# daxiongpro/EPNet

Measured on AMD Instinct MI355X. Metric: SA-stack points/sec per GPU (16384-pt KITTI scene) + % HBM roofline, higher is better.
Workload: dtype f32

## Files before the change

### epnet_amd/_lib.py

```python
import contextlib
import ctypes
import os

_HERE = os.path.dirname(os.path.abspath(__file__))
LIB_PATH = os.environ.get("EPNET_HIP_LIB") or os.path.join(_HERE, "lib", "libepnet_hip.so")

_vp = ctypes.c_void_p
_i = ctypes.c_int
_f = ctypes.c_float
_d = ctypes.c_double
_sz = ctypes.c_size_t
_i64 = ctypes.c_int64

SIGNATURES = {
    "epnet_abi_version": (_i, []),
    "epnet_strerror": (ctypes.c_char_p, [_i]),
    "epnet_last_hip_error": (ctypes.c_char_p, []),
    "epnet_set_tuning": (_i, [ctypes.c_char_p, _i]),
    "epnet_get_tuning": (_i, [ctypes.c_char_p, ctypes.POINTER(_i)]),
    "epnet_furthest_point_sampling": (_i, [_i, _i, _i, _vp, _vp, _vp, _vp]),
    "epnet_gather_points": (_i, [_i, _i, _i, _i, _vp, _vp, _vp, _vp]),
    "epnet_gather_points_grad": (_i, [_i, _i, _i, _i, _vp, _vp, _vp, _vp]),
    "epnet_ball_query": (_i, [_i, _i, _i, _f, _i, _vp, _vp, _vp, _vp]),
    "epnet_ball_query_workspace_bytes": (_sz, [_i, _i, _i]),
# ... 28 lines not shown
    "epnet_three_interpolate_grad_det": (_i, [_i, _i, _i, _i, _vp, _vp, _vp, _vp, _vp, _sz, _vp]),
    "epnet_feature_gather_grad_det_workspace_bytes": (_sz, [_i, _i, _i, _i]),
    "epnet_feature_gather_grad_det": (_i, [_i, _i, _i, _i, _i, _i, _vp, _vp, _vp, _vp, _sz, _vp]),
    "epnet_group_linear_grad_w_det_workspace_bytes": (_sz, [_i, _i, _i, _i]),
    "epnet_group_linear_grad_w_det": (_i, [_i, _i, _i, _i, _i, _vp, _vp, _vp, _vp, _vp, _vp, _sz, _vp]),
    "epnet_pool_max": (_i, [ctypes.c_longlong, _i, _vp, _vp, _vp, _vp]),
    "epnet_pool_max_grad": (_i, [ctypes.c_longlong, _i, _vp, _vp, _vp, _vp]),
    "epnet_scene_index_bytes": (_sz, [_i, _i]),
    "epnet_scene_index_build": (_i, [_i, _i, _vp, _vp, _sz, _vp]),
    "epnet_scene_index_build_gathered": (_i, [_i, _i, _i, _vp, _vp, _vp, _vp, _sz, _vp]),
    "epnet_furthest_point_sampling_indexed": (_i, [_i, _i, _i, _vp, _vp, _sz, _vp, _vp, _vp]),
    "epnet_sample_centres": (_i, [_i, _i, _i, _vp, _vp, _sz, _vp, _vp, _vp, _vp]),
    "epnet_sample_centres_chain": (_i, [_i, _i, _i, _vp, _vp, _sz, _vp, _vp, _vp, _vp, _vp, _i, _vp]),
    "epnet_group_concat_multi": (_i, [_i, _i, _i, _i, _i, _vp, _vp, _vp, _vp, _vp, _vp, _i, _vp]),
    "epnet_ball_query_indexed_multi": (_i, [_i, _i, _i, _i, _vp, _vp, _vp, _vp, _vp, _sz, _vp, _vp]),
    "epnet_ball_query_ordered": (_i, [_i, _i, _i, _i, _vp, _vp, _vp, _vp, _vp, _sz, _vp, _sz, _vp, _vp]),
    "epnet_three_nn_indexed": (_i, [_i, _i, _i, _vp, _vp, _vp, _sz, _vp, _sz, _vp, _vp, _vp]),
    "epnet_ball_query_indexed": (_i, [_i, _i, _i, _f, _i, _vp, _vp, _vp, _sz, _vp, _vp]),
    "epnet_boxes_overlap_bev": (_i, [_i, _vp, _i, _vp, _vp, _vp]),
    "epnet_boxes_iou_bev": (_i, [_i, _vp, _i, _vp, _vp, _vp]),
    "epnet_boxes_iou3d": (_i, [_i, _vp, _i, _vp, _vp, _vp]),
    "epnet_boxes_iou3d_pairs": (_i, [_i, _vp, _vp, _vp, _vp]),
    "epnet_aug_roi_by_noise": (_i, [_i, _i, _f, _vp, _vp, _vp, _vp, _vp, _vp, _vp, _vp]),
    "epnet_rpn_proposals_workspace_bytes": (_sz, [_i, _i, _i, _i]),
    "epnet_rpn_proposals": (_i, [_i, _i, _vp, _vp, _vp, _i, _i, _i, _f, _i, _vp, _sz, _vp, _vp, _vp, _vp]),
    "epnet_rcnn_detections_workspace_bytes": (_sz, [_i, _i]),
    "epnet_rcnn_detections": (_i, [_i, _i, _vp, _vp, _vp, _f, _f, _vp, _sz, _vp, _vp, _vp, _vp]),
    "epnet_nms_workspace_bytes": (_sz, [_i]),
    "epnet_nms": (_i, [_vp, _i, _f, _vp, _sz, _vp, _vp, _vp]),
    "epnet_nms_normal": (_i, [_vp, _i, _f, _vp, _sz, _vp, _vp, _vp]),
# ... 61 lines not shown
```

### epnet_amd/csrc/ball_query.hip

```cpp

#include "common.h"
#include "dpp.h"
#include "spatial.h"

namespace epnet {

constexpr int kBqTile = 2048;
constexpr int kBqThreads = 256;

template <int CPW>
__global__ __launch_bounds__(kBqThreads) void ball_query_kernel(int n, int m, float radius2, int nsample,
                                                                const float *__restrict__ new_xyz,
                                                                const float *__restrict__ xyz,
                                                                int *__restrict__ idx) {
    __shared__ float tile[kBqTile * 3];
    const int lane = threadIdx.x & 63, wave = threadIdx.x >> 6;
    const int bs = blockIdx.y;
    xyz += (size_t)bs * n * 3;
    new_xyz += (size_t)bs * m * 3;
    idx += (size_t)bs * m * nsample;

    const int c0 = (blockIdx.x * (kBqThreads / 64) + wave) * CPW;
    float cx[CPW], cy[CPW], cz[CPW];
    int cnt[CPW], first[CPW];
// ... 332 lines not shown
            for (int s0 = 0; s0 < nqc; s0 += 16) {
                const int slot = s0 + (lane >> 2);
                int bid = 0;
                bool bnear = false;
                if (slot < nqc) {
                    bid = quads[slot] * 4 + (lane & 3);
                    bnear = box_near(boxes + bid * 6, cx, cy, cz, r2);
                }
                scan_buckets(__ballot(bnear), [&](int l) { return __builtin_amdgcn_readlane(bid, l); });
            }
            __builtin_amdgcn_wave_barrier();
        }
    }
}

__device__ __forceinline__ void bq_emit_list(int lane, const int *hits, int cnt, int nsample, int *__restrict__ out) {
    __builtin_amdgcn_wave_barrier();
    const int mine = lane < cnt ? hits[lane] : 0x7fffffff;
    int rank = 0;
    for (int j = 0; j < cnt; ++j) rank += __builtin_amdgcn_readlane(mine, j) < mine ? 1 : 0;
    if (lane < cnt && rank < nsample) out[rank] = mine;
    int first = 0;
    if (cnt) first = __builtin_amdgcn_readlane(mine, (int)__builtin_ctzll(__ballot(lane < cnt && rank == 0)));
    for (int l = cnt + lane; l < nsample; l += 64) out[l] = first;
}

template <int RM>
__device__ __forceinline__ int bq_select_smallest(int lane, int *hits, int cnt, int nsample, int np) {
    __builtin_amdgcn_wave_barrier();
    int key[RM];
#pragma unroll
    for (int r = 0; r < RM; ++r) key[r] = (r * 64 < cnt && r * 64 + lane < cnt) ? hits[r * 64 + lane] : 0x7fffffff;
    int lo = 0, hi = np;
    while (hi - lo > 1) {
        const int mid = (lo + hi) >> 1;
        int c = 0;
#pragma unroll
        for (int r = 0; r < RM; ++r)
            if (r * 64 < cnt) c += (int)__popcll(__ballot(key[r] < mid));
// ... 1 lines not shown
        else lo = mid;
    }
    __builtin_amdgcn_wave_barrier();
    int base = 0;
#pragma unroll
    for (int r = 0; r < RM; ++r)
        if (r * 64 < cnt) {
            const bool sel = key[r] < hi;
            const unsigned long long sm = __ballot(sel);
            if (sel) hits[base + popc_below(sm)] = key[r];
            base += (int)__popcll(sm);
        }
    return hi;
}

template <int DPL>
__device__ __forceinline__ void bq_bitmap_search(int lane, int np, float r2, int nsample, float cx, float cy, float cz,
                                                 const float4 *__restrict__ sorted, const float *__restrict__ boxes,
                                                 const float *__restrict__ qboxes, int *__restrict__ out, unsigned *bits,
                                                 int *quads) {
#pragma unroll
    for (int w = 0; w < DPL; ++w) bits[lane * DPL + w] = 0u;
    __builtin_amdgcn_wave_barrier();
    bq_walk<DPL>(lane, np, r2, cx, cy, cz, sorted, boxes, qboxes, quads, [&](const float4 &p, float d2) {
        if (d2 < r2) {
            const int k = __float_as_int(p.w);
            atomicOr(&bits[k >> 5], 1u << (k & 31));
        }
    });
    __builtin_amdgcn_wave_barrier();
    int bc = 0;
#pragma unroll 8
    for (int i = 0; i < DPL; ++i) bc += __popc(bits[lane * DPL + i]);
    const int incl = wave_inclusive_scan(bc);
    const int total = __builtin_amdgcn_readlane(incl, 63);
    int pos = incl - bc;
    int mine_first = 0x7fffffff;
    if (bc > 0 && (pos < nsample || pos == 0)) {
        for (int i = 0; i < DPL; ++i) {
            unsigned ww = bits[lane * DPL + i];
            if (ww && mine_first == 0x7fffffff) mine_first = (lane * DPL + i) * 32 + (int)__builtin_ctz(ww);
            while (ww && pos < nsample) {
                const int bit = (int)__builtin_ctz(ww);
                ww &= ww - 1u;
                out[pos++] = (lane * DPL + i) * 32 + bit;
            }
            if (pos >= nsample) break;
        }
    }
    const unsigned long long have = __ballot(bc > 0);
    int first = 0;
    if (have) first = __builtin_amdgcn_readlane(mine_first, (int)__builtin_ctzll(have));
    for (int l = total + lane; l < nsample; l += 64) out[l] = first;
}

template <int K>
struct BqScales {
    float r2[K];
    int nsample[K];
    int *idx[K];
};

template <int DPL, int K>
__global__ __launch_bounds__(kQThreads) void bq_query_kernel(int np, int m, BqScales<K> sc,
                                                             const float *__restrict__ new_xyz,
                                                             const float4 *__restrict__ sorted,
                                                             const float *__restrict__ boxes,
                                                             const float *__restrict__ qboxes,
                                                             const float4 *__restrict__ order, int npc) {
    __shared__ unsigned s_bits[kQThreads / 64][64 * DPL];
    __shared__ int s_quads[kQThreads / 64][64];
    __shared__ int s_hits[kQThreads / 64][K][64];
    const int lane = threadIdx.x & 63, wave = threadIdx.x >> 6;
    int wg_x, bs;
    xcd_scene_map(wg_x, bs);
    int ci = wg_x * (kQThreads / 64) + wave;
// ... 28 lines not shown
                cnt[k] += (int)__popcll(hm);
            }
        }
    });
#pragma unroll
    for (int k = 0; k < K; ++k) {
        int *out = sc.idx[k] + ((size_t)bs * m + ci) * sc.nsample[k];
        if (cnt[k] <= 64)
            bq_emit_list(lane, s_hits[wave][k], cnt[k], sc.nsample[k], out);
        else
            bq_bitmap_search<DPL>(lane, np, sc.r2[k], sc.nsample[k], cx, cy, cz, sorted, boxes, qboxes, out, s_bits[wave],
                                  s_quads[wave]);
    }
}

template <int DPL, int K, bool kStream>
__global__ __launch_bounds__(kQThreads) void bq_query2_kernel(int np, int m, BqScales<K> sc,
                                                              const float *__restrict__ new_xyz,
                                                              const float4 *__restrict__ sorted,
                                                              const float *__restrict__ boxes,
                                                              const float *__restrict__ qboxes,
                                                              const float4 *__restrict__ order, int npc) {
    constexpr int kRowsPerStep = 2;
    constexpr int CAP = kStream ? (K == 1 ? 512 : 256) : 64, kStepAppends = kRowsPerStep * 64;
    static_assert(CAP % 64 == 0, "the lists are selected and emitted in whole waves");
    static_assert(!kStream || CAP - kStepAppends >= 64,
                  "a cut list keeps nsample <= 64 entries (the launcher streams for nsample <= 64 only) and must take a step's appends");
    constexpr int kBitWords = kStream ? 0 : 64 * DPL;
    __shared__ unsigned s_pool[kQThreads / 64][kBitWords + 2 * K * CAP];
    __shared__ int s_quads[kQThreads / 64][2][64];
    const int lane = threadIdx.x & 63, wave = threadIdx.x >> 6;
    int wg_x, bs;
    xcd_scene_map(wg_x, bs);
    const int ci0 = (wg_x * (kQThreads / 64) + wave) * 2;
    if (ci0 >= m) return;
    const bool two = ci0 + 1 < m;
    sorted += (size_t)bs * np;
// ... 133 lines not shown
#pragma unroll
        for (int k = 0; k < K; ++k) {
            int *out = sc.idx[k] + ((size_t)bs * m + (e ? out1 : out0)) * sc.nsample[k];
            int *hits = hits_of + (e * K + k) * CAP;
            if constexpr (kStream) {
                if (cnt[e][k] > 64) {
                    bq_select_smallest<CAP / 64>(lane, hits, cnt[e][k], sc.nsample[k], np);
                    cnt[e][k] = sc.nsample[k];
#ifdef EPNET_BQ_STATS
                    st_sel = true;
#endif
                }
                bq_emit_list(lane, hits, cnt[e][k], sc.nsample[k], out);
            } else {
                if (cnt[e][k] <= 64) {
                    bq_emit_list(lane, hits, cnt[e][k], sc.nsample[k], out);
                } else {
#ifdef EPNET_BQ_STATS
                    st_again = true;
#endif
                    bq_bitmap_search<DPL>(lane, np, sc.r2[k], sc.nsample[k], cx, cy, cz, sorted, boxes, qboxes, out, s_pool[wave],
                                          s_quads[wave][0]);
                }
            }
        }
    }
#ifdef EPNET_BQ_STATS
    {
        const unsigned long long st_3 = __builtin_amdgcn_s_memtime();
        if (lane == 0) {
            const int o = st_again ? 8 : (st_sel ? 4 : 0);
            atomicAdd(&g_bq_stats[o + 0], 1ull);
            atomicAdd(&g_bq_stats[o + 1], st_1 - st_0);
            atomicAdd(&g_bq_stats[o + 2], st_3 - st_1);
            atomicAdd(&g_bq_stats[o + 3], (unsigned long long)st_rows);
            atomicMax(&g_bq_stats[12], st_3 - st_0);
        }
    }
#endif
// ... 27 lines not shown
                                hipStream_t s, int n_src, const int *src_idx, float *gathered) {
    if (n <= 4096) {
        constexpr int T = 256, cells = 1 << 12;
        const size_t stage = (np & 255) == 0 ? (size_t)(np / 4 < 512 ? np / 4 : 512) * sizeof(float4) : 0;
        hipLaunchKernelGGL((bq_index_kernel<T, 12>), dim3(b), dim3(T), (size_t)(cells + cells / (cells / T) + 64) * sizeof(int) + stage, s,
                           n, np, xyz, sorted, boxes, qboxes, n_src, src_idx, gathered);
    } else {
        constexpr int T = 1024, cells = 1 << 14;
        const size_t stage = (n <= T * 16 && (np & 255) == 0) ? (size_t)(np / 4) * sizeof(float4) : 0;
        hipLaunchKernelGGL((bq_index_kernel<T, 14>), dim3(b), dim3(T), (size_t)(cells + cells / (cells / T) + 64) * sizeof(int) + stage, s,
                           n, np, xyz, sorted, boxes, qboxes, n_src, src_idx, gathered);
    }
    return check_launch("spatial index");
}

template <int K>
static int bq_query_launch(int b, int np, int m, const BqScales<K> &sc, const float *new_xyz, const float4 *sorted,
                           hipStream_t s, const float4 *order = nullptr, int npc = 0) {
    const float *boxes = (const float *)(sorted + (size_t)b * np);
    const float *qboxes = boxes + (size_t)b * (np / 64) * 6;
    const int pair_force = tuning(kBqPair);
    const bool pair = pair_force >= 0 ? pair_force != 0 : (long long)b * m >= 65536;
    if (pair) {
        dim3 grid(div_up(div_up(m, 2), kQThreads / 64), b);
        const int stream_force = tuning(kBqStream);
        bool stream = stream_force >= 0 ? stream_force != 0 : np > 16384;
        for (int k = 0; k < K; ++k) stream = stream && sc.nsample[k] <= 64;
#define EPNET_BQ2(D_)                                                                                                                   \
    do {                                                                                                                                \
        if (stream)                                                                                                                     \
            hipLaunchKernelGGL((bq_query2_kernel<D_, K, true>), grid, dim3(kQThreads), 0, s, np, m, sc, new_xyz, sorted, boxes, qboxes,   \
                               order, npc);                                                                                             \
        else                                                                                                                            \
            hipLaunchKernelGGL((bq_query2_kernel<D_, K, false>), grid, dim3(kQThreads), 0, s, np, m, sc, new_xyz, sorted, boxes,         \
                               qboxes, order, npc);                                                                                     \
    } while (0)
        switch (np / 2048) {
            case 1: EPNET_BQ2(1); break;
            case 2: EPNET_BQ2(2); break;
            case 4: EPNET_BQ2(4); break;
            case 8: EPNET_BQ2(8); break;
            case 16: EPNET_BQ2(16); break;
// ... 73 lines not shown
            const int rc = epnet_ball_query_indexed(b, n, m, radii[k], nsamples[k], new_xyz, xyz, index, index_bytes, idx[k], stream);
            if (rc) return rc;
        }
        return EPNET_OK;
    }
    EPNET_REQUIRE(new_xyz && idx[0] && idx[1]);
    if (index_bytes < need) return EPNET_ENOMEM;
    EPNET_REQUIRE(b <= 65535);
    BqScales<2> sc;
    for (int k = 0; k < 2; ++k) {
        sc.r2[k] = radii[k] * radii[k];
        sc.nsample[k] = nsamples[k];
        sc.idx[k] = idx[k];
    }
    return bq_query_launch<2>(b, scene_index_np(n), m, sc, new_xyz, (const float4 *)index, (hipStream_t)stream);
}

extern "C" int epnet_ball_query_ordered(int b, int n, int m, int nscales, const float *radii, const int *nsamples,
                                        const float *new_xyz, const float *xyz, const void *index, size_t index_bytes,
                                        const void *centre_index, size_t centre_index_bytes, int *const *idx,
                                        epnet_stream_t stream) {
    EPNET_REQUIRE(nscales >= 0 && (nscales == 0 || (radii && nsamples && idx)));
    const size_t need = scene_index_bytes(b, n), need_c = scene_index_bytes(b, m);
    bool ordered = (nscales == 1 || nscales == 2) && need != 0 && need_c != 0 && index && centre_index && m > 0;
    for (int k = 0; ordered && k < nscales; ++k) ordered = nsamples[k] > 0 && idx[k] != nullptr;
    const int force = tuning(kBqOrdered);
    if (force >= 0 ? force == 0 : n <= 16384) ordered = false;
    if (!ordered) return epnet_ball_query_indexed_multi(b, n, m, nscales, radii, nsamples, new_xyz, xyz, index, index_bytes, idx, stream);
    if (index_bytes < need || centre_index_bytes < need_c) return EPNET_ENOMEM;
    EPNET_REQUIRE(b <= 65535);
// ... 50 lines not shown
```

### epnet_amd/csrc/group.hip

```cpp

#include "common.h"
#include "spatial.h"
#include "runsum.h"

namespace epnet {

constexpr int kGThreads = 256;
constexpr int kGChan = 16;

__global__ __launch_bounds__(kGThreads) void gather_rows_vec4_kernel(int c, int n, int p, size_t ostride,
                                                                     const float *__restrict__ points,
                                                                     const int *__restrict__ idx,
                                                                     float *__restrict__ out) {
    int wg_x, wg_y, bs;
    xcd_scene_map3(wg_x, wg_y, bs);
    const int c0 = wg_y * kGChan;
    const int q4 = wg_x * kGThreads + threadIdx.x;
    if (q4 * 4 >= p) return;
    const int4 id = *reinterpret_cast<const int4 *>(idx + (size_t)bs * p + (size_t)q4 * 4);
    const int cend = min(c, c0 + kGChan);
    const float *src = points + ((size_t)bs * c + c0) * n;
    float *dst = out + (size_t)bs * ostride + (size_t)c0 * p + (size_t)q4 * 4;
#pragma unroll 4
    for (int ci = c0; ci < cend; ++ci) {
// ... 109 lines not shown
            v.x = row[id.x];
            v.y = row[id.y];
            v.z = row[id.z];
            v.w = row[id.w];
            store_stream(dst, v.x, v.y, v.z, v.w);
            row += n;
            dst += p;
        }
    }
}

#ifndef EPNET_GATHER_LDS2_UNROLL
#define EPNET_GATHER_LDS2_UNROLL 1
#endif
constexpr long long kGatherLds2MinPositions = 3 * kGLdsThreads * 4;
template <bool QUAD>
__global__ __launch_bounds__(kGLdsThreads) void gather_rows_lds2_kernel(int c, int n, int rows, const float *__restrict__ points,
                                                                        int p0, size_t ostride0, const int *__restrict__ idx0,
                                                                        float *__restrict__ out0, int p1, size_t ostride1,
                                                                        const int *__restrict__ idx1, float *__restrict__ out1) {
    extern __shared__ float s_rows[];
    int wg_x, bs;
    xcd_scene_map(wg_x, bs);
    const int c0 = wg_x * rows;
    const int nr = min(rows, c - c0);
    const float *src = points + ((size_t)bs * c + c0) * n;
    const int total = nr * n;
    if (QUAD) {
        stage_quads(src, nr >> 2, n, reinterpret_cast<float4 *>(s_rows), kGLdsThreads);
    } else if ((n & 3) == 0 && ((uintptr_t)src & 15) == 0) {
        const float4 *src4 = reinterpret_cast<const float4 *>(src);
        float4 *dst4 = reinterpret_cast<float4 *>(s_rows);
        EPNET_STAGE_PRAGMA
        for (int e = threadIdx.x; e < total / 4; e += kGLdsThreads) dst4[e] = src4[e];
    } else {
        for (int e = threadIdx.x; e < total; e += kGLdsThreads) s_rows[e] = src[e];
    }
    __syncthreads();
// ... 429 lines not shown

extern "C" int epnet_group_points(int b, int c, int n, int npoints, int nsample, const float *points, const int *idx,
                                  float *out, epnet_stream_t stream) {
    EPNET_REQUIRE(b >= 0 && c >= 0 && n >= 0 && npoints >= 0 && nsample >= 0);
    return launch_gather_rows(b, c, n, (long long)npoints * nsample, points, idx, out, (hipStream_t)stream,
                              "group_points");
}

extern "C" int epnet_group_points_grad(int b, int c, int n, int npoints, int nsample, const float *grad_out,
                                       const int *idx, float *grad_points, epnet_stream_t stream) {
    EPNET_REQUIRE(b >= 0 && c >= 0 && n >= 0 && npoints >= 0 && nsample >= 0);
    return launch_scatter_rows(b, c, n, (long long)npoints * nsample, grad_out, idx, grad_points, (hipStream_t)stream,
                               "group_points_grad");
}

static int launch_group_xyz(int b, int n, int npoints, int nsample, long long p, size_t ostride, const float *xyz,
                            const float *new_xyz, const int *idx, float *out, hipStream_t s) {
    if (nsample % 4 == 0 && (((uintptr_t)idx | (uintptr_t)out) % 16 == 0) && (ostride % 4 == 0))
        hipLaunchKernelGGL(group_xyz_centred_vec4_kernel, dim3((unsigned)div_up64(p / 4, kGThreads), b), dim3(kGThreads), 0, s, n,
                           npoints, nsample, ostride, xyz, new_xyz, idx, out);
    else
        hipLaunchKernelGGL(group_xyz_centred_kernel, dim3((unsigned)div_up64(p, kGThreads), b), dim3(kGThreads), 0, s, n, npoints,
                           nsample, ostride, xyz, new_xyz, idx, out);
    return check_launch("group_concat xyz");
}

extern "C" int epnet_group_concat(int b, int c, int n, int npoints, int nsample, const float *xyz, const float *new_xyz,
                                  const float *features, const int *idx, float *out, int use_xyz, epnet_stream_t stream) {
    EPNET_REQUIRE(b >= 0 && c >= 0 && n >= 0 && npoints >= 0 && nsample >= 0);
    EPNET_REQUIRE(use_xyz || c > 0);
    const long long p = (long long)npoints * nsample;
    if (b == 0 || p == 0) return EPNET_OK;
    EPNET_REQUIRE(idx && out && (c == 0 || features) && (!use_xyz || (xyz && new_xyz)));
    EPNET_REQUIRE(n > 0);
    if (p > 0x7fffffffll || b > 65535) return EPNET_ELIMIT;
    hipStream_t s = (hipStream_t)stream;
    const int ch0 = use_xyz ? 3 : 0;
    const size_t ostride = (size_t)(ch0 + c) * (size_t)p;
    if (use_xyz) {
        int rc = launch_group_xyz(b, n, npoints, nsample, p, ostride, xyz, new_xyz, idx, out, s);
        if (rc) return rc;
    }
    if (c == 0) return EPNET_OK;
    return launch_gather_rows(b, c, n, p, features, idx, out + (size_t)ch0 * p, s, "group_concat features", ostride);
}

extern "C" size_t epnet_group_concat_workspace_bytes(int b, int c, int n, int npoints, int nsample) {
    return gather_pm_ws_bytes(b, c, n, (long long)npoints * nsample);
}

extern "C" int epnet_group_concat_ws(int b, int c, int n, int npoints, int nsample, const float *xyz, const float *new_xyz,
                                     const float *features, const int *idx, float *out, int use_xyz, void *workspace,
                                     size_t workspace_bytes, epnet_stream_t stream) {
    const long long p = (long long)npoints * nsample;
    const size_t need = gather_pm_ws_bytes(b, c, n, p);
    if (need == 0 || !workspace || ((uintptr_t)workspace & 15))
        return epnet_group_concat(b, c, n, npoints, nsample, xyz, new_xyz, features, idx, out, use_xyz, stream);
    if (workspace_bytes < need) return EPNET_ENOMEM;
    EPNET_REQUIRE(b >= 0 && n > 0 && npoints >= 0 && nsample >= 0 && features && idx && out && (!use_xyz || (xyz && new_xyz)));
    if (p > 0x7fffffffll || b > 65535) return EPNET_ELIMIT;
    const int ch0 = use_xyz ? 3 : 0;
    const size_t ostride = (size_t)(ch0 + c) * (size_t)p;
    if (use_xyz) {
        int rc = launch_group_xyz(b, n, npoints, nsample, p, ostride, xyz, new_xyz, idx, out, (hipStream_t)stream);
        if (rc) return rc;
    }
    return launch_gather_rows_pm(b, c, n, p, features, idx, out + (size_t)ch0 * p, ostride, workspace, (hipStream_t)stream,
                                 "group_concat features");
}

extern "C" int epnet_group_concat_multi(int b, int c, int n, int npoints, int nscales, const int *nsamples, const float *xyz,
                                        const float *new_xyz, const float *features, const int *const *idx, float *const *out,
                                        int use_xyz, epnet_stream_t stream) {
    EPNET_REQUIRE(nscales >= 0 && (nscales == 0 || (nsamples && idx && out)));
    hipStream_t s = (hipStream_t)stream;
    const int ch0 = use_xyz ? 3 : 0;
    constexpr int kLdsBudget = EPNET_GATHER_LDS_BUDGET_KB * 1024;
    bool fused = nscales == 2 && c >= 8 && b > 0 && n > 0 && npoints > 0 && (size_t)n * 4 <= (size_t)kLdsBudget && features && b <= 65535;
    int rows = 0;
// ... 11 lines not shown
                    (((uintptr_t)idx[k] | (uintptr_t)out[k]) % 16 == 0) && ((size_t)(ch0 + c) * (size_t)p) % 4 == 0;
            p_both += p;
        }
        fused = fused && p_both >= kGatherLds2MinPositions;
        fused = fused && (long long)b * div_up(c, rows) >= 512;
    }
    if (!fused) {
        for (int k = 0; k < nscales; ++k) {
            const int rc = epnet_group_concat(b, c, n, npoints, nsamples[k], xyz, new_xyz, features, idx[k], out[k], use_xyz, stream);
            if (rc) return rc;
        }
        return EPNET_OK;
    }
    size_t ostride[2];
    int pk[2];
    for (int k = 0; k < 2; ++k) {
        pk[k] = npoints * nsamples[k];
        ostride[k] = (size_t)(ch0 + c) * (size_t)pk[k];
        if (!use_xyz) continue;
        EPNET_REQUIRE(xyz && new_xyz);
        const long long p = pk[k];
        if (nsamples[k] % 4 == 0)
            hipLaunchKernelGGL(group_xyz_centred_vec4_kernel, dim3((unsigned)div_up64(p / 4, kGThreads), b), dim3(kGThreads), 0, s,
                               n, npoints, nsamples[k], ostride[k], xyz, new_xyz, idx[k], out[k]);
        else
            hipLaunchKernelGGL(group_xyz_centred_kernel, dim3((unsigned)div_up64(p, kGThreads), b), dim3(kGThreads), 0, s, n,
                               npoints, nsamples[k], ostride[k], xyz, new_xyz, idx[k], out[k]);
        const int rc = check_launch("group_concat_multi xyz");
        if (rc) return rc;
    }
    if (quad)
        hipLaunchKernelGGL(gather_rows_lds2_kernel<true>, dim3(div_up(c, rows), b), dim3(kGLdsThreads), (size_t)rows * n * 4, s, c, n,
                           rows, features, pk[0], ostride[0], idx[0], out[0] + (size_t)ch0 * pk[0], pk[1], ostride[1], idx[1],
                           out[1] + (size_t)ch0 * pk[1]);
    else
        hipLaunchKernelGGL(gather_rows_lds2_kernel<false>, dim3(div_up(c, rows), b), dim3(kGLdsThreads), (size_t)rows * n * 4, s, c, n,
                           rows, features, pk[0], ostride[0], idx[0], out[0] + (size_t)ch0 * pk[0], pk[1], ostride[1], idx[1],
                           out[1] + (size_t)ch0 * pk[1]);
    return check_launch("group_concat_multi");
}

extern "C" int epnet_group_concat_grad(int b, int c, int n, int npoints, int nsample, const float *grad_out, const int *idx,
                                       float *grad_features, int use_xyz, epnet_stream_t stream) {
    EPNET_REQUIRE(b >= 0 && c >= 0 && n >= 0 && npoints >= 0 && nsample >= 0);
// ... 92 lines not shown
```

### epnet_amd/csrc/spatial.h

```cpp
#pragma once
#include "common.h"

namespace epnet {

__device__ __forceinline__ unsigned spread10(unsigned v) {
    v &= 0x3FFu;
    v = (v | (v << 16)) & 0x030000FFu;
    v = (v | (v << 8)) & 0x0300F00Fu;
    v = (v | (v << 4)) & 0x030C30C3u;
    v = (v | (v << 2)) & 0x09249249u;
    return v;
}

__device__ __forceinline__ unsigned morton30(float px, float py, float pz, const float (&lo)[3], float scale) {
    const unsigned ix = (unsigned)fminf((px - lo[0]) * scale, 1023.f);
    const unsigned iy = (unsigned)fminf((py - lo[1]) * scale, 1023.f);
    const unsigned iz = (unsigned)fminf((pz - lo[2]) * scale, 1023.f);
    return spread10(ix) | (spread10(iy) << 1) | (spread10(iz) << 2);
}

__device__ __forceinline__ void bitonic_sort_lds(unsigned long long *keys, int np) {
    const int q = threadIdx.x, T = blockDim.x;
    for (int k2 = 2; k2 <= np; k2 <<= 1)
        for (int j2 = k2 >> 1; j2 > 0; j2 >>= 1) {
// ... 153 lines not shown
    return np;
}
inline size_t scene_index_bytes(int b, int n) {
    if (b <= 0 || n < 1024 || n > 65536) return 0;
    const size_t np = (size_t)scene_index_np(n);
    return (size_t)b * (np * sizeof(float4) + (np / 64 + np / 256) * 6 * sizeof(float) + (n > 16384 ? np * sizeof(float) : 0));
}
inline float *scene_index_sampling_scratch(int b, int n, void *index) {
    const size_t np = (size_t)scene_index_np(n);
    return (float *)((char *)index + (size_t)b * (np * sizeof(float4) + (np / 64 + np / 256) * 6 * sizeof(float)));
}

int spatial_index_launch(int b, int n, int np, const float *xyz, float4 *sorted, float *boxes, float *qboxes, hipStream_t s,
                         int n_src = 0, const int *src_idx = nullptr, float *gathered = nullptr);

}
```

### epnet_amd/pointnet2_cuda.py

```python
import torch

from . import _lib
from ._tensor import dev_ptr, need, on_device_of, writes

_F, _I = torch.float32, torch.int32


def _deterministic():
    return torch.are_deterministic_algorithms_enabled()


def _det_call(l, name, ws_bytes, like, args, s, what):
    ws = torch.empty((max(int(ws_bytes), 1),), dtype=torch.uint8, device=like.device)
    _lib.check(getattr(l, "epnet_%s_det" % name)(*args, ws.data_ptr(), int(ws_bytes), s), "%s (deterministic)" % what)


@writes("idx")
def ball_query_wrapper(b, n, m, radius, nsample, new_xyz, xyz, idx):
    pn, px, pi = dev_ptr(new_xyz, "new_xyz", _F), dev_ptr(xyz, "xyz", _F), dev_ptr(idx, "idx", _I)
    need(new_xyz, b * m * 3, "new_xyz"); need(xyz, b * n * 3, "xyz"); need(idx, b * m * nsample, "idx")
    l = _lib.lib()
    ws_bytes = l.epnet_ball_query_workspace_bytes(b, n, m)
    with on_device_of(xyz) as s:
        if ws_bytes:
# ... 215 lines not shown
    need(new_xyz, b * m * 3, "new_xyz"); need(xyz, b * n * 3, "xyz")
    k = len(radii)
    assert len(nsamples) == k and len(idxs) == k
    ptrs = []
    for ns, t in zip(nsamples, idxs):
        ptrs.append(dev_ptr(t, "idx", _I))
        need(t, b * m * ns, "idx")
    px, nb = _index_args(index, xyz)
    c_r = (ctypes.c_float * k)(*[float(r) for r in radii])
    c_n = (ctypes.c_int * k)(*[int(x) for x in nsamples])
    c_p = (ctypes.c_void_p * k)(*ptrs)
    with on_device_of(xyz) as s:
        _lib.check(_lib.lib().epnet_ball_query_indexed_multi(b, n, m, k, ctypes.cast(c_r, ctypes.c_void_p),
                                                             ctypes.cast(c_n, ctypes.c_void_p), pn, pxyz, px, nb,
                                                             ctypes.cast(c_p, ctypes.c_void_p), s), "ball_query")
    return 1


@writes("idxs")
def ball_query_ordered_wrapper(b, n, m, radii, nsamples, new_xyz, xyz, index, centre_index, idxs):
    import ctypes
    pn, pxyz = dev_ptr(new_xyz, "new_xyz", _F), dev_ptr(xyz, "xyz", _F)
    need(new_xyz, b * m * 3, "new_xyz"); need(xyz, b * n * 3, "xyz")
    k = len(radii)
    assert len(nsamples) == k and len(idxs) == k
    ptrs = []
    for ns, t in zip(nsamples, idxs):
        ptrs.append(dev_ptr(t, "idx", _I))
        need(t, b * m * ns, "idx")
    px, nb = _index_args(index, xyz)
# ... 191 lines not shown
```

### epnet_amd/sa_stack.py

```python
import os

import torch

from . import pointnet2_cuda as ext

RPN_NPOINTS = (4096, 1024, 256, 64)
RPN_RADII = ((0.1, 0.5), (0.5, 1.0), (1.0, 2.0), (2.0, 4.0))
RPN_NSAMPLES = ((16, 32), (16, 32), (16, 32), (16, 32))
RPN_FEAT_CHANNELS = (0, 96, 256, 512)
RPN_FP = ((1024, 64, 256), (512, 256, 1024), (512, 1024, 4096), (256, 4096, 16384))


CONFIGS = {
    2: dict(n=16384, npoints=RPN_NPOINTS, radii=RPN_RADII, nsamples=RPN_NSAMPLES, feat_channels=RPN_FEAT_CHANNELS),
    5: dict(n=65536, npoints=(16384,), radii=((0.5,),), nsamples=((64,),), feat_channels=(64,)),
}


def sa_algorithmic_bytes(n=16384, npoints=RPN_NPOINTS, nsamples=RPN_NSAMPLES, feat_channels=RPN_FEAT_CHANNELS):
    out = {"fps": 0, "gather": 0, "ball_query": 0, "group_xyz": 0, "group_feat": 0}
    cur = n
    for lvl, m in enumerate(npoints):
        out["fps"] += cur * 12 + m * 4
        out["gather"] += m * 4 + 3 * cur * 4 + 3 * m * 4
# ... 47 lines not shown
        elif env_q == 2 or (env_q == 1 and with_fp):
            chosen = every
        elif env_q == 1 and batch * n >= 240 * 16384:
            chosen = every - {0}
        else:
            chosen = frozenset()
        self.s_query_levels = chosen & every
        self.queries_in_s = self.s_query_levels == every
        self.chain = bool(int(os.environ.get("EPNET_SA_CHAIN", "1"))) and fused_sampling
        self.fuse_gather = bool(int(os.environ.get("EPNET_SA_FUSE_GATHER", "1")))
        self._deferred = None
        self.s_first = bool(int(os.environ.get("EPNET_SA_S_FIRST", "0" if self.s_query_levels else "1")))
        self.tail_scales = int(os.environ.get("EPNET_SA_TAIL_SCALES", "0"))
        self.multi_query = bool(int(os.environ.get("EPNET_SA_MULTI_QUERY", "1")))
        self.multi_group = bool(int(os.environ.get("EPNET_SA_MULTI_GROUP", "1")))
        self.ordered_query = bool(int(os.environ.get("EPNET_SA_ORDERED_QUERY", "1")))
        self.side = None
        self.npoints, self.radii, self.nsamples, self.feat_channels = npoints, radii, nsamples, feat_channels
        self.with_fp, self.fp = with_fp, fp
        dev = torch.device(device)
        g = torch.Generator().manual_seed(seed)
        f32, i32 = torch.float32, torch.int32
        self.levels = []
        cur = n
        for lvl, m in enumerate(npoints):
            c = feat_channels[lvl]
            index_bytes = ext.scene_index_bytes(batch, cur) if shared_index else 0
            L = {
                "n": cur, "m": m, "c": c,
                "xyz_t_sets": [torch.empty((batch, 3, cur), dtype=f32, device=dev) for _ in range(self.ring if not fused else 1)],
# ... 158 lines not shown
        own = L["sets"][parity].get("centre_index")
        if own is not None:
            ext.scene_index_build_wrapper(self.batch, L["m"], L["sets"][parity]["new_xyz"], own)
        return own

    def _group_scales(self, L, cur_xyz, parity):
        if self.fused and self.multi_group and len(L["scales"]) > 1:
            ext.group_concat_multi_wrapper(self.batch, L["c"], L["n"], L["m"], [S["ns"] for S in L["scales"]], cur_xyz,
                                           L["sets"][parity]["new_xyz"], L["features"], [self._idx(S, parity) for S in L["scales"]],
                                           [S["grouped"] for S in L["scales"]], True)
        else:
            for S in L["scales"]:
                self._group_scale(L, S, cur_xyz, parity)

    def _group_level(self, L, cur_xyz, parity):
        self._query_level(L, cur_xyz, parity)
        self._group_scales(L, cur_xyz, parity)

    def _side_stream(self, device):
        if self.side is None:
            self.side = torch.cuda.Stream(device=device)
        return self.side

    def run(self, xyz):
        main = torch.cuda.current_stream(xyz.device)
        side = self._side_stream(xyz.device) if self.overlap else None
        cur_xyz = xyz
        built = False
        for lvl, L in enumerate(self.levels):
            new_xyz = self._sample_level(L, cur_xyz, 0, index_built=built)
# ... 217 lines not shown
```

### include/epnet_ops.h

```cpp
#ifndef EPNET_OPS_H
#define EPNET_OPS_H

#include <stddef.h>
#include <stdint.h>

#ifdef __cplusplus
extern "C" {
#endif

#define EPNET_ABI_VERSION 1

#define EPNET_OK 0
#define EPNET_EINVAL (-1)
#define EPNET_ELAUNCH (-2)
#define EPNET_ENOMEM (-3)
#define EPNET_ELIMIT (-4)

typedef void *epnet_stream_t;

int epnet_abi_version(void);
const char *epnet_strerror(int code);
const char *epnet_last_hip_error(void);

int epnet_set_tuning(const char *name, int value);
// ... 103 lines not shown
int epnet_furthest_point_sampling_indexed(int b, int n, int m, const float *xyz, void *index,
                                          size_t index_bytes, float *temp, int *idx, epnet_stream_t stream);
int epnet_sample_centres(int b, int n, int m, const float *xyz, void *index, size_t index_bytes, float *temp,
                         int *idx, float *new_xyz, epnet_stream_t stream);
int epnet_sample_centres_chain(int b, int n, int m, const float *xyz, void *index, size_t index_bytes, float *temp,
                               int *idx, float *new_xyz, const int *prefix_in, int *prefix_out, int prefix_cap,
                               epnet_stream_t stream);
int epnet_three_nn_indexed(int b, int n, int m, const float *unknown, const float *known, const void *unknown_index,
                           size_t unknown_index_bytes, const void *known_index, size_t known_index_bytes, float *dist2,
                           int *idx, epnet_stream_t stream);
int epnet_ball_query_indexed(int b, int n, int m, float radius, int nsample, const float *new_xyz, const float *xyz,
                             const void *index, size_t index_bytes, int *idx, epnet_stream_t stream);
int epnet_ball_query_indexed_multi(int b, int n, int m, int nscales, const float *radii, const int *nsamples,
                                   const float *new_xyz, const float *xyz, const void *index, size_t index_bytes,
                                   int *const *idx, epnet_stream_t stream);
int epnet_ball_query_ordered(int b, int n, int m, int nscales, const float *radii, const int *nsamples, const float *new_xyz,
                             const float *xyz, const void *index, size_t index_bytes, const void *centre_index,
                             size_t centre_index_bytes, int *const *idx, epnet_stream_t stream);


int epnet_boxes_overlap_bev(int num_a, const float *boxes_a, int num_b, const float *boxes_b,
                            float *ans_overlap, epnet_stream_t stream);

int epnet_boxes_iou_bev(int num_a, const float *boxes_a, int num_b, const float *boxes_b,
                        float *ans_iou, epnet_stream_t stream);

int epnet_boxes_iou3d(int num_a, const float *boxes_a, int num_b, const float *boxes_b, float *ans_iou3d,
                      epnet_stream_t stream);

int epnet_boxes_iou3d_pairs(int k, const float *boxes_a, const float *boxes_b, float *ans_iou3d, epnet_stream_t stream);
// ... 64 lines not shown
```

Baseline: 1.373 billion.

## Fuse xyz grouping into ball query and into multi-scale feature gather

Adds a ball-query kernel variant that, for two-scale levels without features, writes the centred grouped xyz directly from the in-register neighbour lists, so no separate group-xyz pass re-reads the indices. For levels with features, the xyz grouping is folded into the LDS row-gather kernel as one extra workgroup per scene that stages the scene points in shared memory. This removes kernel launches and index re-reads, at the cost of extra register pressure (occupancy hint of 8) and an imbalanced final workgroup in the gather grid.

```diff
diff --git a/epnet_amd/_lib.py b/epnet_amd/_lib.py
--- a/epnet_amd/_lib.py
+++ b/epnet_amd/_lib.py
@@ -66,6 +66,7 @@
     "epnet_sample_centres_chain": (_i, [_i, _i, _i, _vp, _vp, _sz, _vp, _vp, _vp, _vp, _vp, _i, _vp]),
     "epnet_group_concat_multi": (_i, [_i, _i, _i, _i, _i, _vp, _vp, _vp, _vp, _vp, _vp, _i, _vp]),
     "epnet_ball_query_indexed_multi": (_i, [_i, _i, _i, _i, _vp, _vp, _vp, _vp, _vp, _sz, _vp, _vp]),
+    "epnet_ball_query_group_xyz_multi": (_i, [_i, _i, _i, _i, _vp, _vp, _vp, _vp, _vp, _sz, _vp, _vp, _vp, _vp]),
     "epnet_ball_query_ordered": (_i, [_i, _i, _i, _i, _vp, _vp, _vp, _vp, _vp, _sz, _vp, _sz, _vp, _vp]),
     "epnet_three_nn_indexed": (_i, [_i, _i, _i, _vp, _vp, _vp, _sz, _vp, _sz, _vp, _vp, _vp]),
     "epnet_ball_query_indexed": (_i, [_i, _i, _i, _f, _i, _vp, _vp, _vp, _sz, _vp, _vp]),
diff --git a/epnet_amd/csrc/ball_query.hip b/epnet_amd/csrc/ball_query.hip
--- a/epnet_amd/csrc/ball_query.hip
+++ b/epnet_amd/csrc/ball_query.hip
@@ -1,3 +1,5 @@
+
+#include <type_traits>
 
 #include "common.h"
 #include "dpp.h"
@@ -370,15 +372,24 @@
     }
 }
 
-__device__ __forceinline__ void bq_emit_list(int lane, const int *hits, int cnt, int nsample, int *__restrict__ out) {
+template <bool kRow = false>
+__device__ __forceinline__ void bq_emit_list(int lane, const int *hits, int cnt, int nsample, int *__restrict__ out,
+                                             int *row = nullptr) {
     __builtin_amdgcn_wave_barrier();
     const int mine = lane < cnt ? hits[lane] : 0x7fffffff;
     int rank = 0;
     for (int j = 0; j < cnt; ++j) rank += __builtin_amdgcn_readlane(mine, j) < mine ? 1 : 0;
-    if (lane < cnt && rank < nsample) out[rank] = mine;
+    if constexpr (kRow) __builtin_amdgcn_wave_barrier();
+    if (lane < cnt && rank < nsample) {
+        out[rank] = mine;
+        if constexpr (kRow) row[rank] = mine;
+    }
     int first = 0;
     if (cnt) first = __builtin_amdgcn_readlane(mine, (int)__builtin_ctzll(__ballot(lane < cnt && rank == 0)));
-    for (int l = cnt + lane; l < nsample; l += 64) out[l] = first;
+    for (int l = cnt + lane; l < nsample; l += 64) {
+        out[l] = first;
+        if constexpr (kRow) row[l] = first;
+    }
 }
 
 template <int RM>
@@ -410,11 +421,11 @@
     return hi;
 }
 
-template <int DPL>
+template <int DPL, bool kRow = false>
 __device__ __forceinline__ void bq_bitmap_search(int lane, int np, float r2, int nsample, float cx, float cy, float cz,
                                                  const float4 *__restrict__ sorted, const float *__restrict__ boxes,
                                                  const float *__restrict__ qboxes, int *__restrict__ out, unsigned *bits,
-                                                 int *quads) {
+                                                 int *quads, int *row = nullptr) {
 #pragma unroll
     for (int w = 0; w < DPL; ++w) bits[lane * DPL + w] = 0u;
     __builtin_amdgcn_wave_barrier();
@@ -439,6 +450,7 @@
             while (ww && pos < nsample) {
                 const int bit = (int)__builtin_ctz(ww);
                 ww &= ww - 1u;
+                if constexpr (kRow) row[pos] = (lane * DPL + i) * 32 + bit;
                 out[pos++] = (lane * DPL + i) * 32 + bit;
             }
             if (pos >= nsample) break;
@@ -447,7 +459,10 @@
     const unsigned long long have = __ballot(bc > 0);
     int first = 0;
     if (have) first = __builtin_amdgcn_readlane(mine_first, (int)__builtin_ctzll(have));
-    for (int l = total + lane; l < nsample; l += 64) out[l] = first;
+    for (int l = total + lane; l < nsample; l += 64) {
+        out[l] = first;
+        if constexpr (kRow) row[l] = first;
+    }
 }
 
 template <int K>
@@ -456,6 +471,16 @@
     int nsample[K];
     int *idx[K];
 };
+
+template <int K>
+struct BqGroup {
+    const float *xyz;
+    int n;
+    float *out[K];
+    long long ostride[K];
+    int inv1[K], inv2[K];
+};
+struct BqNoGroup {};
 
 template <int DPL, int K>
 __global__ __launch_bounds__(kQThreads) void bq_query_kernel(int np, int m, BqScales<K> sc,
@@ -514,13 +539,15 @@
     }
 }
 
-template <int DPL, int K, bool kStream>
-__global__ __launch_bounds__(kQThreads) void bq_query2_kernel(int np, int m, BqScales<K> sc,
+template <int DPL, int K, bool kStream, bool kGroup = false>
+__global__ __launch_bounds__(kQThreads, kGroup ? 8 : 0) void bq_query2_kernel(int np, int m, BqScales<K> sc,
                                                               const float *__restrict__ new_xyz,
                                                               const float4 *__restrict__ sorted,
                                                               const float *__restrict__ boxes,
                                                               const float *__restrict__ qboxes,
-                                                              const float4 *__restrict__ order, int npc) {
+                                                              const float4 *__restrict__ order, int npc,
+                                                              std::conditional_t<kGroup, BqGroup<K>, BqNoGroup> grp = {}) {
+    static_assert(!kGroup || !kStream, "the grouping mode reads the rows out of the 64-entry lists");
     constexpr int kRowsPerStep = 2;
     constexpr int CAP = kStream ? (K == 1 ? 512 : 256) : 64, kStepAppends = kRowsPerStep * 64;
     static_assert(CAP % 64 == 0, "the lists are selected and emitted in whole waves");
@@ -684,15 +711,46 @@
                 bq_emit_list(lane, hits, cnt[e][k], sc.nsample[k], out);
             } else {
                 if (cnt[e][k] <= 64) {
-                    bq_emit_list(lane, hits, cnt[e][k], sc.nsample[k], out);
+                    bq_emit_list<kGroup>(lane, hits, cnt[e][k], sc.nsample[k], out, hits);
                 } else {
 #ifdef EPNET_BQ_STATS
                     st_again = true;
 #endif
-                    bq_bitmap_search<DPL>(lane, np, sc.r2[k], sc.nsample[k], cx, cy, cz, sorted, boxes, qboxes, out, s_pool[wave],
-                                          s_quads[wave][0]);
+                    bq_bitmap_search<DPL, kGroup>(lane, np, sc.r2[k], sc.nsample[k], cx, cy, cz, sorted, boxes, qboxes, out,
+                                                  s_pool[wave], s_quads[wave][0], hits);
                 }
             }
+        }
+    }
+    if constexpr (kGroup) {
+        __builtin_amdgcn_wave_barrier();
+        constexpr int kIt = 3;
+        const float *pts = grp.xyz + (size_t)bs * grp.n * 3;
+        float v[K][kIt];
+        unsigned off[K][kIt];
+#pragma unroll
+        for (int k = 0; k < K; ++k) {
+            const int ns = sc.nsample[k], P = two ? 2 * ns : ns, tot = 3 * P, invp = two ? grp.inv2[k] : grp.inv1[k];
+#pragma unroll
+            for (int it = 0; it < kIt; ++it) {
+                v[k][it] = 0.f;
+                off[k][it] = ~0u;
+                if (it * 64 < tot) {
+                    const int i = it * 64 + lane, ii = i < tot ? i : 0;
+                    const int ch = (ii * invp) >> 16, t = ii - ch * P, e = t >= ns ? 1 : 0, j = t - e * ns;
+                    const int id = hits_of[(e * K + k) * CAP + j];
+                    const float c = e ? (ch == 0 ? bx_ : ch == 1 ? by_ : bz_) : (ch == 0 ? ax : ch == 1 ? ay : az);
+                    v[k][it] = pts[(unsigned)(id * 3 + ch)] - c;
+                    if (i < tot) off[k][it] = (unsigned)((ch * m + (e ? out1 : out0)) * ns + j);
+                }
+            }
+        }
+#pragma unroll
+        for (int k = 0; k < K; ++k) {
+            float *dst = grp.out[k] + (size_t)bs * grp.ostride[k];
+#pragma unroll
+            for (int it = 0; it < kIt; ++it)
+                if (off[k][it] != ~0u) __builtin_nontemporal_store(v[k][it], dst + off[k][it]);
         }
     }
 #ifdef EPNET_BQ_STATS
@@ -750,18 +808,49 @@
     return check_launch("spatial index");
 }
 
+static void bq_query_route(int b, int np, int m, const int *nsample, int nscales, bool &pair, bool &stream) {
+    const int pair_force = tuning(kBqPair);
+    pair = pair_force >= 0 ? pair_force != 0 : (long long)b * m >= 65536;
+    const int stream_force = tuning(kBqStream);
+    stream = stream_force >= 0 ? stream_force != 0 : np > 16384;
+    for (int k = 0; k < nscales; ++k) stream = stream && nsample[k] <= 64;
+}
+
+static bool bq_group_applies(int b, int np, int m, const int *nsample) {
+    bool pair, stream;
+    bq_query_route(b, np, m, nsample, 2, pair, stream);
+    if (!pair || stream || np > 16384) return false;
+    for (int k = 0; k < 2; ++k)
+        if (nsample[k] < 1 || nsample[k] > 32 || 3ll * m * nsample[k] > 0x7fffffffll) return false;
+    return true;
+}
+
 template <int K>
 static int bq_query_launch(int b, int np, int m, const BqScales<K> &sc, const float *new_xyz, const float4 *sorted,
-                           hipStream_t s, const float4 *order = nullptr, int npc = 0) {
+                           hipStream_t s, const float4 *order = nullptr, int npc = 0, const BqGroup<K> *grp = nullptr) {
     const float *boxes = (const float *)(sorted + (size_t)b * np);
     const float *qboxes = boxes + (size_t)b * (np / 64) * 6;
-    const int pair_force = tuning(kBqPair);
-    const bool pair = pair_force >= 0 ? pair_force != 0 : (long long)b * m >= 65536;
+    bool pair, stream;
+    bq_query_route(b, np, m, sc.nsample, K, pair, stream);
+    if constexpr (K == 2) {
+        if (grp) {
+            dim3 grid(div_up(div_up(m, 2), kQThreads / 64), b);
+#define EPNET_BQ2G(D_)                                                                                                                 \
+    hipLaunchKernelGGL((bq_query2_kernel<D_, 2, false, true>), grid, dim3(kQThreads), 0, s, np, m, sc, new_xyz, sorted, boxes, qboxes, \
+                       order, npc, *grp)
+            switch (np / 2048) {
+                case 1: EPNET_BQ2G(1); break;
+                case 2: EPNET_BQ2G(2); break;
+                case 4: EPNET_BQ2G(4); break;
+                case 8: EPNET_BQ2G(8); break;
+                default: return EPNET_EINVAL;
+            }
+#undef EPNET_BQ2G
+            return check_launch("ball_query query + xyz grouping");
+        }
+    }
     if (pair) {
         dim3 grid(div_up(div_up(m, 2), kQThreads / 64), b);
-        const int stream_force = tuning(kBqStream);
-        bool stream = stream_force >= 0 ? stream_force != 0 : np > 16384;
-        for (int k = 0; k < K; ++k) stream = stream && sc.nsample[k] <= 64;
 #define EPNET_BQ2(D_)                                                                                                                   \
     do {                                                                                                                                \
         if (stream)                                                                                                                     \
@@ -865,6 +954,52 @@
         sc.idx[k] = idx[k];
     }
     return bq_query_launch<2>(b, scene_index_np(n), m, sc, new_xyz, (const float4 *)index, (hipStream_t)stream);
+}
+
+extern "C" int epnet_ball_query_group_xyz_multi(int b, int n, int m, int nscales, const float *radii, const int *nsamples,
+                                                const float *new_xyz, const float *xyz, const void *index, size_t index_bytes,
+                                                int *const *idx, float *const *out, const size_t *ostride,
+                                                epnet_stream_t stream) {
+    EPNET_REQUIRE(nscales >= 0 && (nscales == 0 || (radii && nsamples && idx && out && ostride)));
+    EPNET_REQUIRE(b >= 0 && n >= 0 && m >= 0);
+    for (int k = 0; k < nscales; ++k) {
+        EPNET_REQUIRE(nsamples[k] >= 0);
+        EPNET_REQUIRE(ostride[k] >= (size_t)3 * (size_t)m * (size_t)nsamples[k]);
+    }
+    const size_t need = scene_index_bytes(b, n);
+    bool fused = nscales == 2 && need != 0 && index && m > 0 && b <= 65535;
+    if (fused) {
+        EPNET_REQUIRE(new_xyz && xyz && idx[0] && idx[1] && out[0] && out[1]);
+        if (index_bytes < need) return EPNET_ENOMEM;
+        fused = bq_group_applies(b, scene_index_np(n), m, nsamples);
+    }
+    if (fused) {
+        BqScales<2> sc;
+        BqGroup<2> grp;
+        grp.xyz = xyz;
+        grp.n = n;
+        for (int k = 0; k < 2; ++k) {
+            sc.r2[k] = radii[k] * radii[k];
+            sc.nsample[k] = nsamples[k];
+            sc.idx[k] = idx[k];
+            grp.out[k] = out[k];
+            grp.ostride[k] = (long long)ostride[k];
+            grp.inv1[k] = (65536 + nsamples[k] - 1) / nsamples[k];
+            grp.inv2[k] = (65536 + 2 * nsamples[k] - 1) / (2 * nsamples[k]);
+        }
+        return bq_query_launch<2>(b, scene_index_np(n), m, sc, new_xyz, (const float4 *)index, (hipStream_t)stream, nullptr, 0, &grp);
+    }
+    int rc = epnet_ball_query_indexed_multi(b, n, m, nscales, radii, nsamples, new_xyz, xyz, index, index_bytes, idx, stream);
+    if (rc) return rc;
+    for (int k = 0; k < nscales; ++k) {
+        const long long p = (long long)m * nsamples[k];
+        if (b == 0 || p == 0) continue;
+        EPNET_REQUIRE(idx[k] && out[k] && xyz && new_xyz && n > 0);
+        if (p > 0x7fffffffll || b > 65535) return EPNET_ELIMIT;
+        rc = group_xyz_launch(b, n, m, nsamples[k], p, ostride[k], xyz, new_xyz, idx[k], out[k], (hipStream_t)stream);
+        if (rc) return rc;
+    }
+    return EPNET_OK;
 }
 
 extern "C" int epnet_ball_query_ordered(int b, int n, int m, int nscales, const float *radii, const int *nsamples,
diff --git a/epnet_amd/csrc/group.hip b/epnet_amd/csrc/group.hip
--- a/epnet_amd/csrc/group.hip
+++ b/epnet_amd/csrc/group.hip
@@ -1,3 +1,5 @@
+
+#include <type_traits>
 
 #include "common.h"
 #include "spatial.h"
@@ -147,14 +149,62 @@
 #define EPNET_GATHER_LDS2_UNROLL 1
 #endif
 constexpr long long kGatherLds2MinPositions = 3 * kGLdsThreads * 4;
-template <bool QUAD>
+#ifndef EPNET_GATHER_XYZ_CHUNK
+#define EPNET_GATHER_XYZ_CHUNK 1
+#endif
+struct GatherXyz {
+    const float *xyz, *new_xyz;
+    int npoints, ns0, ns1;
+};
+struct GatherNoXyz {};
+
+__device__ __forceinline__ void gather_xyz_chunk(const GatherXyz &g, int n, int bs, float *s_rows, int p0, size_t ostride0,
+                                                 const int *__restrict__ idx0, float *__restrict__ out0, int p1, size_t ostride1,
+                                                 const int *__restrict__ idx1, float *__restrict__ out1) {
+    float4 *s_pt = reinterpret_cast<float4 *>(s_rows);
+    const float4 *src = reinterpret_cast<const float4 *>(g.xyz + (size_t)bs * n * 3);
+    for (int e = threadIdx.x; e < (n >> 2); e += kGLdsThreads) {
+        const float4 a = src[e * 3], b4 = src[e * 3 + 1], cc = src[e * 3 + 2];
+        s_pt[e * 4 + 0] = make_float4(a.x, a.y, a.z, 0.f);
+        s_pt[e * 4 + 1] = make_float4(a.w, b4.x, b4.y, 0.f);
+        s_pt[e * 4 + 2] = make_float4(b4.z, b4.w, cc.x, 0.f);
+        s_pt[e * 4 + 3] = make_float4(cc.y, cc.z, cc.w, 0.f);
+    }
+    __syncthreads();
+    const float *centres = g.new_xyz + (size_t)bs * g.npoints * 3;
+#pragma unroll 1
+    for (int set = 0; set < 2; ++set) {
+        const int p = set ? p1 : p0, ns = set ? g.ns1 : g.ns0;
+        const int *ix = (set ? idx1 : idx0) + (size_t)bs * p;
+        float *dst_base = (set ? out1 : out0) + (size_t)bs * (set ? ostride1 : ostride0) - 3 * (size_t)p;
+        for (int q = threadIdx.x * 4; q < p; q += kGLdsThreads * 4) {
+            const int4 id = *reinterpret_cast<const int4 *>(ix + q);
+            const float *ce = centres + (q / ns) * 3;
+            const float cx = ce[0], cy = ce[1], cz = ce[2];
+            const float4 v0 = s_pt[id.x], v1 = s_pt[id.y], v2 = s_pt[id.z], v3 = s_pt[id.w];
+            float *dst = dst_base + q;
+            store_stream(dst, v0.x - cx, v1.x - cx, v2.x - cx, v3.x - cx);
+            store_stream(dst + p, v0.y - cy, v1.y - cy, v2.y - cy, v3.y - cy);
+            store_stream(dst + 2 * (size_t)p, v0.z - cz, v1.z - cz, v2.z - cz, v3.z - cz);
+        }
+    }
+}
+
+template <bool QUAD, bool XYZ = false>
 __global__ __launch_bounds__(kGLdsThreads) void gather_rows_lds2_kernel(int c, int n, int rows, const float *__restrict__ points,
                                                                         int p0, size_t ostride0, const int *__restrict__ idx0,
                                                                         float *__restrict__ out0, int p1, size_t ostride1,
-                                                                        const int *__restrict__ idx1, float *__restrict__ out1) {
+                                                                        const int *__restrict__ idx1, float *__restrict__ out1,
+                                                                        std::conditional_t<XYZ, GatherXyz, GatherNoXyz> gx = {}) {
     extern __shared__ float s_rows[];
     int wg_x, bs;
     xcd_scene_map(wg_x, bs);
+    if constexpr (XYZ) {
+        if (wg_x == (int)gridDim.x - 1) {
+            gather_xyz_chunk(gx, n, bs, s_rows, p0, ostride0, idx0, out0, p1, ostride1, idx1, out1);
+            return;
+        }
+    }
     const int c0 = wg_x * rows;
     const int nr = min(rows, c - c0);
     const float *src = points + ((size_t)bs * c + c0) * n;
@@ -614,7 +664,7 @@
                                "group_points_grad");
 }
 
-static int launch_group_xyz(int b, int n, int npoints, int nsample, long long p, size_t ostride, const float *xyz,
+int epnet::group_xyz_launch(int b, int n, int npoints, int nsample, long long p, size_t ostride, const float *xyz,
                             const float *new_xyz, const int *idx, float *out, hipStream_t s) {
     if (nsample % 4 == 0 && (((uintptr_t)idx | (uintptr_t)out) % 16 == 0) && (ostride % 4 == 0))
         hipLaunchKernelGGL(group_xyz_centred_vec4_kernel, dim3((unsigned)div_up64(p / 4, kGThreads), b), dim3(kGThreads), 0, s, n,
@@ -638,7 +688,7 @@
     const int ch0 = use_xyz ? 3 : 0;
     const size_t ostride = (size_t)(ch0 + c) * (size_t)p;
     if (use_xyz) {
-        int rc = launch_group_xyz(b, n, npoints, nsample, p, ostride, xyz, new_xyz, idx, out, s);
+        int rc = group_xyz_launch(b, n, npoints, nsample, p, ostride, xyz, new_xyz, idx, out, s);
         if (rc) return rc;
     }
     if (c == 0) return EPNET_OK;
@@ -662,7 +712,7 @@
     const int ch0 = use_xyz ? 3 : 0;
     const size_t ostride = (size_t)(ch0 + c) * (size_t)p;
     if (use_xyz) {
-        int rc = launch_group_xyz(b, n, npoints, nsample, p, ostride, xyz, new_xyz, idx, out, (hipStream_t)stream);
+        int rc = group_xyz_launch(b, n, npoints, nsample, p, ostride, xyz, new_xyz, idx, out, (hipStream_t)stream);
         if (rc) return rc;
     }
     return launch_gather_rows_pm(b, c, n, p, features, idx, out + (size_t)ch0 * p, ostride, workspace, (hipStream_t)stream,
@@ -704,11 +754,13 @@
     }
     size_t ostride[2];
     int pk[2];
+    if (use_xyz) EPNET_REQUIRE(xyz && new_xyz);
+    const bool xyz_chunk = EPNET_GATHER_XYZ_CHUNK && use_xyz && (size_t)n * 16 <= (size_t)kLdsBudget && (n & 3) == 0 && nsamples[0] % 4 == 0 &&
+                           nsamples[1] % 4 == 0 && ((uintptr_t)xyz & 15) == 0;
     for (int k = 0; k < 2; ++k) {
         pk[k] = npoints * nsamples[k];
         ostride[k] = (size_t)(ch0 + c) * (size_t)pk[k];
-        if (!use_xyz) continue;
-        EPNET_REQUIRE(xyz && new_xyz);
+        if (!use_xyz || xyz_chunk) continue;
         const long long p = pk[k];
         if (nsamples[k] % 4 == 0)
             hipLaunchKernelGGL(group_xyz_centred_vec4_kernel, dim3((unsigned)div_up64(p / 4, kGThreads), b), dim3(kGThreads), 0, s,
@@ -718,6 +770,20 @@
                                npoints, nsamples[k], ostride[k], xyz, new_xyz, idx[k], out[k]);
         const int rc = check_launch("group_concat_multi xyz");
         if (rc) return rc;
+    }
+    if (xyz_chunk) {
+        const GatherXyz gx = {xyz, new_xyz, npoints, nsamples[0], nsamples[1]};
+        const size_t lds = (size_t)rows * n * 4 > (size_t)n * 16 ? (size_t)rows * n * 4 : (size_t)n * 16;
+        const dim3 grid(div_up(c, rows) + 1, b);
+        if (quad)
+            hipLaunchKernelGGL((gather_rows_lds2_kernel<true, true>), grid, dim3(kGLdsThreads), lds, s, c, n, rows, features, pk[0],
+                               ostride[0], idx[0], out[0] + (size_t)ch0 * pk[0], pk[1], ostride[1], idx[1],
+                               out[1] + (size_t)ch0 * pk[1], gx);
+        else
+            hipLaunchKernelGGL((gather_rows_lds2_kernel<false, true>), grid, dim3(kGLdsThreads), lds, s, c, n, rows, features, pk[0],
+                               ostride[0], idx[0], out[0] + (size_t)ch0 * pk[0], pk[1], ostride[1], idx[1],
+                               out[1] + (size_t)ch0 * pk[1], gx);
+        return check_launch("group_concat_multi");
     }
     if (quad)
         hipLaunchKernelGGL(gather_rows_lds2_kernel<true>, dim3(div_up(c, rows), b), dim3(kGLdsThreads), (size_t)rows * n * 4, s, c, n,
diff --git a/epnet_amd/csrc/spatial.h b/epnet_amd/csrc/spatial.h
--- a/epnet_amd/csrc/spatial.h
+++ b/epnet_amd/csrc/spatial.h
@@ -191,4 +191,7 @@
 int spatial_index_launch(int b, int n, int np, const float *xyz, float4 *sorted, float *boxes, float *qboxes, hipStream_t s,
                          int n_src = 0, const int *src_idx = nullptr, float *gathered = nullptr);
 
+int group_xyz_launch(int b, int n, int npoints, int nsample, long long p, size_t ostride, const float *xyz, const float *new_xyz,
+                     const int *idx, float *out, hipStream_t s);
+
 }
diff --git a/epnet_amd/pointnet2_cuda.py b/epnet_amd/pointnet2_cuda.py
--- a/epnet_amd/pointnet2_cuda.py
+++ b/epnet_amd/pointnet2_cuda.py
@@ -253,6 +253,34 @@
         _lib.check(_lib.lib().epnet_ball_query_indexed_multi(b, n, m, k, ctypes.cast(c_r, ctypes.c_void_p),
                                                              ctypes.cast(c_n, ctypes.c_void_p), pn, pxyz, px, nb,
                                                              ctypes.cast(c_p, ctypes.c_void_p), s), "ball_query")
+    return 1
+
+
+@writes("idxs", "outs")
+def ball_query_multi_grouped_wrapper(b, n, m, radii, nsamples, new_xyz, xyz, index, idxs, outs):
+    import ctypes
+    pn, pxyz = dev_ptr(new_xyz, "new_xyz", _F), dev_ptr(xyz, "xyz", _F)
+    need(new_xyz, b * m * 3, "new_xyz"); need(xyz, b * n * 3, "xyz")
+    k = len(radii)
+    assert len(nsamples) == k and len(idxs) == k and len(outs) == k
+    ptrs, optrs, strides = [], [], []
+    for ns, t, o in zip(nsamples, idxs, outs):
+        ptrs.append(dev_ptr(t, "idx", _I)); optrs.append(dev_ptr(o, "out", _F))
+        need(t, b * m * ns, "idx"); need(o, b * 3 * m * ns, "out")
+        if b and (o.numel() % b or o.numel() // b < 3 * m * ns):
+            raise RuntimeError("out: a contiguous (B, 3 + C, M, nsample) tensor is required")
+        strides.append(o.numel() // b if b else 0)
+    px, nb = _index_args(index, xyz)
+    c_r = (ctypes.c_float * k)(*[float(r) for r in radii])
+    c_n = (ctypes.c_int * k)(*[int(x) for x in nsamples])
+    c_p = (ctypes.c_void_p * k)(*ptrs)
+    c_o = (ctypes.c_void_p * k)(*optrs)
+    c_s = (ctypes.c_size_t * k)(*strides)
+    with on_device_of(xyz) as s:
+        _lib.check(_lib.lib().epnet_ball_query_group_xyz_multi(b, n, m, k, ctypes.cast(c_r, ctypes.c_void_p),
+                                                               ctypes.cast(c_n, ctypes.c_void_p), pn, pxyz, px, nb,
+                                                               ctypes.cast(c_p, ctypes.c_void_p), ctypes.cast(c_o, ctypes.c_void_p),
+                                                               ctypes.cast(c_s, ctypes.c_void_p), s), "ball_query")
     return 1
 
 
diff --git a/epnet_amd/sa_stack.py b/epnet_amd/sa_stack.py
--- a/epnet_amd/sa_stack.py
+++ b/epnet_amd/sa_stack.py
@@ -85,6 +85,7 @@
         self.tail_scales = int(os.environ.get("EPNET_SA_TAIL_SCALES", "0"))
         self.multi_query = bool(int(os.environ.get("EPNET_SA_MULTI_QUERY", "1")))
         self.multi_group = bool(int(os.environ.get("EPNET_SA_MULTI_GROUP", "1")))
+        self.fused_xyz = bool(int(os.environ.get("EPNET_SA_FUSED_XYZ", "1")))
         self.ordered_query = bool(int(os.environ.get("EPNET_SA_ORDERED_QUERY", "1")))
         self.side = None
         self.npoints, self.radii, self.nsamples, self.feat_channels = npoints, radii, nsamples, feat_channels
@@ -273,6 +274,14 @@
                 self._group_scale(L, S, cur_xyz, parity)
 
     def _group_level(self, L, cur_xyz, parity):
+        P = L["sets"][parity]
+        if (self.fused_xyz and self.fused and not L["c"] and len(L["scales"]) == 2 and P["index"] is not None
+                and self.multi_query and self.multi_group and L["n"] <= 16384
+                and self.levels.index(L) not in self.s_query_levels):
+            ext.ball_query_multi_grouped_wrapper(self.batch, L["n"], L["m"], [S["radius"] for S in L["scales"]],
+                                                 [S["ns"] for S in L["scales"]], P["new_xyz"], cur_xyz, P["index"],
+                                                 [self._idx(S, parity) for S in L["scales"]], [S["grouped"] for S in L["scales"]])
+            return
         self._query_level(L, cur_xyz, parity)
         self._group_scales(L, cur_xyz, parity)
 
diff --git a/include/epnet_ops.h b/include/epnet_ops.h
--- a/include/epnet_ops.h
+++ b/include/epnet_ops.h
@@ -141,6 +141,9 @@
 int epnet_ball_query_indexed_multi(int b, int n, int m, int nscales, const float *radii, const int *nsamples,
                                    const float *new_xyz, const float *xyz, const void *index, size_t index_bytes,
                                    int *const *idx, epnet_stream_t stream);
+int epnet_ball_query_group_xyz_multi(int b, int n, int m, int nscales, const float *radii, const int *nsamples,
+                                     const float *new_xyz, const float *xyz, const void *index, size_t index_bytes,
+                                     int *const *idx, float *const *out, const size_t *ostride, epnet_stream_t stream);
 int epnet_ball_query_ordered(int b, int n, int m, int nscales, const float *radii, const int *nsamples, const float *new_xyz,
                              const float *xyz, const void *index, size_t index_bytes, const void *centre_index,
                              size_t centre_index_bytes, int *const *idx, epnet_stream_t stream);
```

Result: slower. 1.190 billion (-13.3%).
